# soedinglab/PEnG-motif

Measured on AMD Instinct MI355X. Metric: 4^W pattern z-scores/s + EM PWM-kmer evals/s at W=10; Gbp/s k-mer count, higher is better.
Workload: dtype u32 counts / f32 scores / f32 serial EM sums (f64 tree sums in the throughput EM mode)

## Files before the change

peng-motif_amd/csrc/em.hip:

```cpp
#include "em_serial.h"

namespace pengk {
namespace {
#ifdef PENGK_WG_TRACE
constexpr unsigned WG_TRACE_MAX = 1u << 20;
__device__ unsigned long long g_wg_trace[3 * WG_TRACE_MAX];
__device__ unsigned g_wg_trace_n;
struct WgTrace {
  unsigned long long t0;
  unsigned kernel;
  __device__ __forceinline__ WgTrace(unsigned k) : t0(__builtin_amdgcn_s_memrealtime()), kernel(k) {}
  __device__ __forceinline__ void end(unsigned kind, unsigned wg) const {
    if (threadIdx.x != 0) return;
    const unsigned long long t1 = __builtin_amdgcn_s_memrealtime();
    const unsigned xcc = __builtin_amdgcn_s_getreg((4 << 11) | (0 << 6) | 20) & 0xFu;
    const unsigned i = atomicAdd(&g_wg_trace_n, 1u);
    if (i < WG_TRACE_MAX) {
      g_wg_trace[3 * i] = ((unsigned long long)kernel << 56) | ((unsigned long long)kind << 48) | ((unsigned long long)xcc << 40) | wg;
      g_wg_trace[3 * i + 1] = t0;
      g_wg_trace[3 * i + 2] = t1;
    }
  }
};
#define PENGK_WG_TRACE_BEGIN(k) const WgTrace wg_trace(k)
// ... 347 lines not shown
    constexpr bool LEAN = decltype(lean_tag)::value;
#pragma unroll 1
    for (uint32_t d6 = 0; d6 < 4u; ++d6) {
#pragma unroll
      for (uint32_t d5 = 0; d5 < 4u; ++d5) {
        float s5 = 0.0f;
#pragma unroll
        for (uint32_t d4 = 0; d4 < 4u; ++d4) {
          const uint32_t xl = t + 256u * (d4 + 4u * d5 + 16u * d6);
          float pr = ((p3 * f4_[d4]) * f5_[d5]) * f6_[d6];
#pragma unroll
          for (int p = 7; p < W; ++p) pr = pr * hi[p - 7];
          const float odds = em_div<LEAN>(pr, bgs[xl]);
          const float v = em_div<LEAN>((float)cnt[xl] * saturation, 1 + em_div<LEAN>(saturation, odds));
          out[xl] = v;
          flagged |= __float_as_uint(v) > 0x7F7FFFFFu;
          c4[d4] += v;
          s5 += v;
        }
        c5[d5] += s5;
        c6[d6] += s5;
      }
    }
  };
  if (lean) body(std::true_type{});
  else body(std::false_type{});
  if (flagged) bad[pw] = 1u;
  const float tot = (c6[0] + c6[1]) + (c6[2] + c6[3]);
  auto all = [](float v) {
#pragma unroll
    for (int m = 1; m < 64; m <<= 1) v += __shfl_xor(v, m, 64);
    return v;
  };
#pragma unroll
  for (int a = 0; a < 4; ++a) {
    const float s4 = all(c4[a]), s5 = all(c5[a]), s6 = all(c6[a]);
    if (lane == 0) {
      part[wave][12 + a] = s4;
      part[wave][16 + a] = s5;
      part[wave][20 + a] = s6;
    }
  }
#pragma unroll
  for (int d = 0; d < 3; ++d) {
    float v = tot;
#pragma unroll
    for (int m = 1; m < 64; m <<= 1)
      if (m != (1 << (2 * d)) && m != (2 << (2 * d))) v += __shfl_xor(v, m, 64);
    if ((lane & ~(3u << (2 * d))) == 0u) part[wave][4 * d + (lane >> (2 * d))] = v;
  }
  {
    const float v = all(tot);
    if (lane == 0) part[wave][24] = v;
  }
  __syncthreads();
  if (t < G::CELLS) {
    const uint32_t p = t >> 2, a = t & 3u;
    float* o = sums + (size_t)pw * G::CELLS * G::NBLK;
    if (p <= 6u) {
      float v;
      if (p == 3u) v = part[a][24];
      else {
        const uint32_t at = p <= 2u ? 4u * p + a : 4u * (p - 1u) + a;
        v = (part[0][at] + part[1][at]) + (part[2][at] + part[3][at]);
      }
      o[(size_t)t * G::NBLK + sp] = v;
    } else {
      const float v = (part[0][20 + a] + part[1][20 + a]) + (part[2][20 + a] + part[3][20 + a]);
      o[(size_t)(4u * p + G::high_digit(p, sp)) * G::NBLK + G::high_block(p, sp, a)] = v;
    }
  }
  PENGK_WG_TRACE_END(0, blockIdx.x + gridDim.x * blockIdx.y);
}

template <int W>
__global__ __launch_bounds__(64) void em_block_predict_kernel(const uint32_t* __restrict__ run_now, const uint32_t* __restrict__ bad,
                                                              const float* __restrict__ sums, seqsum::BlockRecord* __restrict__ rec,
                                                              uint32_t skew) {
  using G = BlockGeo<W>;
  const uint32_t pw = blockIdx.y, cell = blockIdx.x, lane = threadIdx.x;
  if (run_now[pw] == 0u || bad[pw]) return;
  constexpr uint32_t PER = G::NBLK / 64u;
  static_assert(G::NBLK % 64u == 0u, "whole lanes");
  const float* in = sums + ((size_t)pw * G::CELLS + cell) * G::NBLK + (size_t)lane * PER;
  seqsum::BlockRecord* out = rec + ((size_t)pw * G::CELLS + cell) * G::NBLK + (size_t)lane * PER;
  double mine = 0.0;
  for (uint32_t i = 0; i < PER; ++i) mine += (double)in[i];
  double before = mine;
#pragma unroll
  for (int d = 1; d < 64; d <<= 1) {
    const double o = __shfl_up(before, d, 64);
    if ((int)lane >= d) before += o;
  }
  before -= mine;
  for (uint32_t i = 0; i < PER; ++i) {
    const double after = before + (double)in[i];
    const uint32_t e = block_binade(before, after, skew, cell * G::NBLK + lane * PER + i);
    seqsum::BlockRecord r;
    r.e = e;
    r.d0 = 0.0f;
    r.d1 = 0.0f;
    r.pad = 0u;
    out[i] = r;
    before = after;
  }
}

constexpr uint32_t SPAN_EVAL_WAVES = 8;
template <int W>
__global__ __launch_bounds__(64 * SPAN_EVAL_WAVES) void em_span_eval_kernel(const uint32_t* __restrict__ run_now, const float* __restrict__ wbuf,
                                                                            seqsum::BlockRecord* __restrict__ rec,
                                                                            const uint32_t* __restrict__ bad, uint32_t n_pwm,
                                                                            const float* __restrict__ sums, uint32_t skew,
                                                                            uint32_t extra_wgs, uint32_t head_blocks) {
  using G = BlockGeo<W>;
  PENGK_WG_TRACE_BEGIN(2);
  const uint32_t lin = blockIdx.x + gridDim.x * blockIdx.y;
  __shared__ __attribute__((aligned(16))) float span[16384];
  const uint32_t t = threadIdx.x, lane = t & 63u;
  const uint32_t wave = (uint32_t)__builtin_amdgcn_readfirstlane((int)(t >> 6));
  if (lin < extra_wgs) {
    constexpr uint32_t XW = (G::CELLS + 3u) / 4u;
    uint32_t pw, xunit;
    if (!group_map(lin, n_pwm, XW, pw, xunit)) return;
    const uint32_t cell = 4u * xunit + wave;
    if (wave >= 4u || cell >= G::CELLS || run_now[pw] == 0u || bad[pw]) return;
    seqsum::lds_float* buf = (seqsum::lds_float*)span + wave * seqsum::BLOCK;
    const float* w = wbuf + (size_t)pw * G::NP;
    seqsum::Row mine;
    seqsum::Stats st;
    float s0 = 0.0f;
    const bool first_position = (cell >> 2) == 0u;
    auto stage = [&](uint32_t b) {
      uint32_t l = lane;
      asm volatile("" : "+v"(l));
      if (first_position) {
        EmTerms0<W> src0{w, cell & 3u};
        src0.bind_stage(l);
        src0.stage(b, l, buf);
      } else {
        EmTerms<W> src{w, cell >> 2, cell & 3u};
        src.bind_stage(l);
        src.stage(b, l, buf);
      }
    };
    stage(0u);
#pragma unroll 1
    for (uint32_t b = 0; b < head_blocks; ++b) {
      asm volatile("s_waitcnt vmcnt(0)" ::: "memory");
      mine.read_staged(buf, lane);
      asm volatile("s_waitcnt lgkmcnt(0)" ::: "memory");
      if (b + 1u < head_blocks) stage(b + 1u);
      s0 = seqsum::fold_block(mine, lane, s0, st);
    }
    if (lane == 0) {
      seqsum::BlockRecord out;
      out.e = seqsum::SUM_BEHIND;
      out.d0 = s0;
      out.d1 = 0.0f;
      out.pad = head_blocks;
      rec[((size_t)pw * G::CELLS + cell) * G::NBLK] = out;
    }
    PENGK_WG_TRACE_END(1, lin);
    return;
  }
  uint32_t pw, sp;
  if (!group_map(lin - extra_wgs, n_pwm, G::SPANS, pw, sp)) return;
  constexpr uint32_t T = 64u * SPAN_EVAL_WAVES, PER = 4096u / T;
  seqsum::f4 v[PER];
  {
    const seqsum::f4* src = reinterpret_cast<const seqsum::f4*>(wbuf + (size_t)pw * G::NP + (size_t)sp * 16384u);
#pragma unroll
    for (uint32_t k = 0; k < PER; ++k) v[k] = src[t + T * k];
  }
  const uint32_t running = run_now[pw];
  const uint32_t flagged = bad[pw];
  constexpr uint32_t TASKS = (G::CELLS + SPAN_EVAL_WAVES - 1u) / SPAN_EVAL_WAVES;
  seqsum::BlockRecord* cells = rec + (size_t)pw * G::CELLS * G::NBLK;
  auto cell_of = [&](uint32_t task) { return (task >> 2) <= 6u ? task : 4u * (task >> 2) + G::high_digit(task >> 2, sp); };
  auto block_of = [&](uint32_t task) { return (task >> 2) <= 6u ? sp : G::high_block(task >> 2, sp, task & 3u); };
  uint32_t binades = seqsum::NO_BINADE;
  if constexpr (G::PREDICT_IN_EVAL) {
    constexpr uint32_t LOADS = G::NBLK / 64u, GROUP = LOADS <= 4u ? TASKS : 2u;
#pragma unroll 1
    for (uint32_t i0 = 0; i0 < TASKS; i0 += GROUP) {
      float part[GROUP], own[GROUP];
#pragma unroll
      for (uint32_t g = 0; g < GROUP; ++g) {
        const uint32_t task = min(wave + SPAN_EVAL_WAVES * (i0 + g), G::CELLS - 1u);
        const uint32_t cell = cell_of(task), b = block_of(task);
        const float* cs = sums + ((size_t)pw * G::CELLS + cell) * G::NBLK;
        float acc = 0.0f;
#pragma unroll
        for (uint32_t c = 0; c < G::NBLK; c += 64u) {
          const float x = cs[c + lane];
          acc += c + lane < b ? x : 0.0f;
        }
        part[g] = acc;
        own[g] = cs[b];
      }
#pragma unroll
      for (uint32_t g = 0; g < GROUP; ++g) {
        const uint32_t i = i0 + g, task = wave + SPAN_EVAL_WAVES * i;
        float acc = part[g];
#pragma unroll
        for (int m = 1; m < 64; m <<= 1) acc += __shfl_xor(acc, m, 64);
        if (i < TASKS && task < G::CELLS) {
          const uint32_t e = block_binade((double)acc, (double)acc + (double)own[g], skew, cell_of(task) * G::NBLK + block_of(task));
          if (lane == i) binades = e;
        }
      }
    }
  } else {
#pragma unroll 1
    for (uint32_t i = 0; i < TASKS; ++i) {
      const uint32_t task = wave + SPAN_EVAL_WAVES * i;
      if (task < G::CELLS) {
        const uint32_t e = cells[(size_t)cell_of(task) * G::NBLK + block_of(task)].e;
        if (lane == i) binades = e;
      }
    }
  }
  if (running == 0 || flagged) return;
  {
    seqsum::f4* dst = reinterpret_cast<seqsum::f4*>(span);
#pragma unroll
    for (uint32_t k = 0; k < PER; ++k) {
      const uint32_t idx = t + T * k;
      dst[SpanLds::slot_of(idx >> 4, idx & 15u)] = v[k];
    }
  }
  __syncthreads();
  PENGK_WG_TRACE_END(2, lin);
#pragma unroll 1
  for (uint32_t task = wave, i = 0; task < G::CELLS; task += SPAN_EVAL_WAVES, ++i) {
    const uint32_t p = task >> 2, j = task & 3u;
    if (block_of(task) < head_blocks) continue;
    seqsum::BlockRecord* r = cells + (size_t)cell_of(task) * G::NBLK + block_of(task);
    const uint32_t e = (uint32_t)__builtin_amdgcn_readlane((int)binades, (int)i);
    if (e == seqsum::NO_BINADE) {
      if (G::PREDICT_IN_EVAL && lane == 0) r->e = seqsum::NO_BINADE;
      continue;
    }
    seqsum::Row mine;
    span_row<W>(span, p, j, lane, mine);
    float d0, d1;
    const bool ok = seqsum::block_increments(mine, lane, seqsum::bases_of_binade(e), d0, d1);
    if (lane == 0) {
      seqsum::BlockRecord out;
      out.e = ok ? e : seqsum::NO_BINADE;
      out.d0 = d0;
      out.d1 = d1;
      out.pad = 0u;
      *r = out;
    }
  }
  PENGK_WG_TRACE_END(0, lin);
}

template <int W>
__global__ __launch_bounds__(64) void em_chain_store_kernel(const uint32_t* __restrict__ run, const uint32_t* __restrict__ bad,
                                                            const float* __restrict__ wbuf, const seqsum::BlockRecord* __restrict__ rec,
                                                            float* __restrict__ cellsum, uint32_t n_pwm,
                                                            unsigned long long* __restrict__ counters) {
  using G = BlockGeo<W>;
  PENGK_WG_TRACE_BEGIN(3);
  const uint32_t lin = blockIdx.x + gridDim.x * blockIdx.y;
  uint32_t pw, cell;
  if (!group_map(lin, n_pwm, G::CELLS, pw, cell)) return;
  __shared__ __attribute__((aligned(16))) float lds[seqsum::WALK_LDS_FLOATS];
  seqsum::WalkCounts wc;
  const uint32_t lane = threadIdx.x;
  const seqsum::BlockRecord* r = rec + ((size_t)pw * G::CELLS + cell) * G::NBLK;
  uint32_t running = run[pw];
  uint32_t flagged = bad[pw];
  uint4 first = reinterpret_cast<const uint4*>(r)[lane];
  asm volatile("" : "+s"(running), "+s"(flagged), "+v"(first.x), "+v"(first.y), "+v"(first.z), "+v"(first.w));
  if (running == 0u) return;
  float s = 0.0f;
  const float* w = wbuf + (size_t)pw * G::NP;
  if (flagged) {
    const uint32_t p = cell >> 2, a = cell & 3u;
    for (uint32_t c = 0; c < (1u << (2 * W - 2)); ++c)
      s += w[((c >> (2u * p)) << (2u * p + 2u)) | (a << (2u * p)) | (c & ((1u << (2u * p)) - 1u))];
  } else if ((cell >> 2) == 0u) {
    EmTerms0<W> src0{w, cell & 3u};
    src0.bind_stage(lane);
    s = seqsum::walk_chain(src0, r, first, G::NBLK, (seqsum::lds_float*)lds, lane, wc);
  } else {
    EmTerms<W> src{w, cell >> 2, cell & 3u};
    src.bind_stage(lane);
    s = seqsum::walk_chain(src, r, first, G::NBLK, (seqsum::lds_float*)lds, lane, wc);
  }
  if (lane == 0) {
    cellsum[(size_t)pw * G::CELLS + cell] = s;
    if (wc.fetched) __hip_atomic_fetch_add(counters + 0, (unsigned long long)wc.fetched, __ATOMIC_RELAXED, __HIP_MEMORY_SCOPE_AGENT);
    if (wc.mispredicted) __hip_atomic_fetch_add(counters + 1, (unsigned long long)wc.mispredicted, __ATOMIC_RELAXED, __HIP_MEMORY_SCOPE_AGENT);
    if (wc.restaged) __hip_atomic_fetch_add(counters + 2, (unsigned long long)wc.restaged, __ATOMIC_RELAXED, __HIP_MEMORY_SCOPE_AGENT);
    if (wc.restaged_waits) __hip_atomic_fetch_add(counters + 3, (unsigned long long)wc.restaged_waits, __ATOMIC_RELAXED, __HIP_MEMORY_SCOPE_AGENT);
  }
  PENGK_WG_TRACE_END(wc.fetched > 255u ? 255u : wc.fetched, lin);
}

template <int W>
__global__ __launch_bounds__(64) void em_serial_finish_kernel(FusedState fs, uint32_t K, float threshold, int max_it) {
  constexpr uint32_t CELLS = 4u * W;
  const uint32_t pw = blockIdx.x, t = threadIdx.x;
  __shared__ __attribute__((aligned(16))) float s_pwm[CELLS], s_old[CELLS];
  const uint32_t running = fs.run[(size_t)((K - 1u) & 1u) * fs.run_stride + pw];
  if (running) {
    const float* prev = ((K - 1u) & 1u) ? fs.pwm1 : fs.pwm0;
    if (t < CELLS) {
      s_old[t] = prev[(size_t)pw * CELLS + t];
      s_pwm[t] = fs.cellsum[(size_t)pw * CELLS + t];
    }
    __syncthreads();
    const float change = finalize_rows<W>(s_pwm, s_old, t);
    if (t < CELLS) fs.pwm0[(size_t)pw * CELLS + t] = s_pwm[t];
    if (t == 0) {
      fs.state[2 * pw] = (int)K;
      fs.state[2 * pw + 1] = !(change <= threshold || (int)K >= max_it);
      fs.change[pw] = change;
    }
  } else {
    const int it = fs.state[2 * pw];
    if ((it & 1) && t < CELLS) fs.pwm0[(size_t)pw * CELLS + t] = fs.pwm1[(size_t)pw * CELLS + t];
  }
  if (t == 0) {
    fs.bad[pw] = 0u;
    fs.bad[(size_t)fs.bad_stride + pw] = 0u;
  }
}

__global__ __launch_bounds__(256) void em_serial_setup_kernel(uint32_t n, int W, float threshold, int max_it, int32_t* __restrict__ state,
                                                             float* __restrict__ change, uint32_t* __restrict__ run,
                                                             unsigned long long* __restrict__ counters, uint32_t* __restrict__ bg_range,
                                                             uint32_t lean, uint32_t* __restrict__ bad, uint32_t bad_words) {
  const uint32_t i = blockIdx.x * 256u + threadIdx.x;
  if (i < (uint32_t)EM_COUNTERS) counters[i] = 0ull;
  if (i == 0) {
    bg_range[0] = lean ? 0xFFFFFFFFu : 0u;
    bg_range[1] = lean ? 0u : 0xFFFFFFFFu;
  }
  for (uint32_t j = i; j < bad_words; j += gridDim.x * 256u) bad[j] = 0u;
  if (i >= n) return;
  const float c0 = (float)W;
  const uint32_t r = !(c0 <= threshold || 0 >= max_it);
  state[2 * i] = 0;
  state[2 * i + 1] = (int32_t)r;
  change[i] = c0;
  run[i] = r;
  run[n + i] = r;
}

template <int W, int HIMAX, bool FAST, int P>
int launch_geo(pengk_ctx* ctx, int64_t n_pwm, float* d_pwms, float saturation, float threshold, int max_it,
               const uint32_t* d_counts, const float* d_bg, int32_t* d_state, float* d_change) {
  using G = EmGeo<W, HIMAX>;
  hipLaunchKernelGGL(em_init_kernel, dim3((unsigned)((n_pwm + 255) / 256)), dim3(256), 0, ctx->stream, (int)n_pwm, W, threshold,
                     max_it, d_state, d_change);
  PENGK_HIP(hipGetLastError());
  const size_t per_pwm = (size_t)G::NB * G::CELLS * sizeof(double);
  const size_t budget = (size_t)256 << 20;
  int64_t batch = (int64_t)(budget / per_pwm);
  if (batch < 1) batch = 1;
  if (batch > n_pwm) batch = n_pwm;
  if (batch > 65535) batch = 65535;
  if (batch > P) batch -= batch % P;
  int rc = ensure_scratch(ctx, (void**)&ctx->d_em_partials, &ctx->em_partials_bytes, (size_t)batch * per_pwm);
  if (rc) return rc;
  if (FAST) {
    const uint32_t np = 1u << (2 * W);
    rc = ensure_scratch(ctx, (void**)&ctx->d_em_tables, &ctx->em_tables_bytes, (size_t)2 * np * sizeof(float));
    if (rc) return rc;
    float* cs = ctx->d_em_tables;
    float* sb = cs + np;
    const unsigned pb = (np + 255) / 256 < 4096u ? (np + 255) / 256 : 4096u;
    hipLaunchKernelGGL(em_prepare_kernel, dim3(pb), dim3(256), 0, ctx->stream, d_counts, d_bg, saturation, np, cs, sb);
    PENGK_HIP(hipGetLastError());
    d_counts = reinterpret_cast<const uint32_t*>(cs);
    d_bg = sb;
  }
  for (int64_t first = 0; first < n_pwm; first += batch) {
    const int64_t nb = n_pwm - first < batch ? n_pwm - first : batch;
    for (int it = 0; it < max_it; ++it) {
      hipLaunchKernelGGL((em_accumulate_kernel<W, HIMAX, FAST, P>), dim3(G::NB, (unsigned)((nb + P - 1) / P)), dim3(256), 0,
                         ctx->stream, d_pwms + (size_t)first * W * 4, d_state + 2 * first, d_counts, d_bg, saturation,
                         ctx->d_em_partials, (int)nb);
      hipLaunchKernelGGL((em_finalize_kernel<W, HIMAX>), dim3((unsigned)nb), dim3(64), 0, ctx->stream,
                         d_pwms + (size_t)first * W * 4, d_state + 2 * first, d_change + first, ctx->d_em_partials, threshold, max_it,
                         (uint32_t*)nullptr, (const float*)nullptr, 0u);
    }
    PENGK_HIP(hipGetLastError());
  }
  return PENGK_OK;
}

#ifdef PENGK_WG_TRACE
}
}
extern "C" __attribute__((visibility("default"))) long long pengk_debug_wg_trace(unsigned long long* out, unsigned max) {
  unsigned n = 0;
  if (hipDeviceSynchronize() != hipSuccess) return -1;
  if (hipMemcpyFromSymbol(&n, HIP_SYMBOL(pengk::g_wg_trace_n), sizeof n) != hipSuccess) return -1;
  const unsigned m = n < max ? n : max;
  if (m && hipMemcpyFromSymbol(out, HIP_SYMBOL(pengk::g_wg_trace), (size_t)m * 3 * sizeof(unsigned long long)) != hipSuccess) return -1;
  const unsigned zero = 0;
  if (hipMemcpyToSymbol(HIP_SYMBOL(pengk::g_wg_trace_n), &zero, sizeof zero) != hipSuccess) return -1;
  return (long long)n;
}
namespace pengk {
namespace {
#endif

#ifdef PENGK_SEQSUM_STATS
}
}
extern "C" __attribute__((visibility("default"))) int pengk_debug_seqsum_stats(unsigned long long* out, int reset) {
  if (hipMemcpyFromSymbol(out, HIP_SYMBOL(pengk::seqsum::g_stats), 12 * sizeof(unsigned long long)) != hipSuccess) return 1;
  if (reset) {
    unsigned long long z[12] = {0};
    if (hipMemcpyToSymbol(HIP_SYMBOL(pengk::seqsum::g_stats), z, sizeof z) != hipSuccess) return 1;
  }
  return 0;
}
namespace pengk {
namespace {
#endif

template <int W>
int launch_serial_ahead(pengk_ctx* ctx, int64_t n_pwm, float* d_pwms, float saturation, float threshold, int max_it,
                        const uint32_t* d_counts, const float* d_bg, int32_t* d_state, float* d_change, size_t budget, bool split) {
  using B = BlockGeo<W>;
  using LG = LookGeo<W>;
  const size_t np = (size_t)1 << (2 * W);
  int lanes = ctx->em_overlap < 1 ? 1 : ctx->em_overlap > MAX_EM_LANES ? MAX_EM_LANES : ctx->em_overlap;
  while (lanes > 1 && n_pwm < 8 * (int64_t)lanes) --lanes;
  const int64_t fit = std::max<int64_t>(1, (int64_t)(budget / lanes / (np * sizeof(float))));
  int64_t batch = fit;
  if (batch * lanes > n_pwm) {
    batch = lanes > 1 ? ((n_pwm + lanes - 1) / lanes + 7) / 8 * 8 : n_pwm;
    if (batch > fit) batch = fit >= 8 ? fit / 8 * 8 : fit;
  }
  if (batch > 16384) batch = 16384;
  const size_t tables_b = (size_t)batch * np * sizeof(float);
  const size_t sums_b = split ? ((size_t)batch * B::CELLS * B::NBLK * sizeof(float) + 255) / 256 * 256 : 0;
  const size_t rec_b = sums_b + ((size_t)batch * B::CELLS * B::NBLK * sizeof(seqsum::BlockRecord) + 255) / 256 * 256;
  const size_t look_b = split ? 0 : ((size_t)batch * LG::WORDS_PER_PWM * sizeof(unsigned long long) + 255) / 256 * 256;
  const size_t flags_at = ((size_t)batch * B::CELLS * sizeof(float) + 255) / 256 * 256;
  const size_t small_b = (flags_at + (size_t)2 * batch * sizeof(uint32_t) + 255) / 256 * 256;
  const size_t run_at = lanes * small_b;
  const size_t pwm1_at = (run_at + (size_t)2 * n_pwm * sizeof(uint32_t) + 255) / 256 * 256;
  int rc = ensure_scratch(ctx, (void**)&ctx->d_em_tables, &ctx->em_tables_bytes, lanes * tables_b);
  if (rc) return rc;
  rc = ensure_scratch(ctx, (void**)&ctx->d_em_partials, &ctx->em_partials_bytes, pwm1_at + (size_t)n_pwm * B::CELLS * sizeof(float));
  if (rc) return rc;
  rc = ensure_scratch(ctx, &ctx->d_em_blocks, &ctx->em_blocks_bytes, lanes * rec_b);
  if (rc) return rc;
  if (look_b) {
    const size_t had = ctx->em_look_bytes;
    rc = ensure_scratch(ctx, &ctx->d_em_look, &ctx->em_look_bytes, lanes * look_b);
    if (rc) return rc;
    if (ctx->em_look_bytes != had || ctx->em_epoch >= 0xFFFF0000u) {
      PENGK_HIP(hipStreamSynchronize(ctx->stream));
      for (int l = 0; l < MAX_EM_LANES - 1; ++l)
        if (ctx->em_streams[l]) PENGK_HIP(hipStreamSynchronize(ctx->em_streams[l]));
      PENGK_HIP(hipMemsetAsync(ctx->d_em_look, 0, ctx->em_look_bytes, ctx->stream));
      ctx->em_epoch = 0;
    }
  }
  if (!ctx->d_em_counters) PENGK_HIP(hipMalloc((void**)&ctx->d_em_counters, (EM_COUNTERS + 1) * sizeof(unsigned long long)));
  uint32_t* bg_range = reinterpret_cast<uint32_t*>(ctx->d_em_counters + EM_COUNTERS);
  char* small = reinterpret_cast<char*>(ctx->d_em_partials);
  uint32_t* run = reinterpret_cast<uint32_t*>(small + run_at);
  float* pwm1 = reinterpret_cast<float*>(small + pwm1_at);
  {
    const uint32_t words = (uint32_t)((run_at - flags_at) / sizeof(uint32_t));
    hipLaunchKernelGGL(em_serial_setup_kernel, dim3((unsigned)((std::max<int64_t>(n_pwm, 1024) + 255) / 256)), dim3(256), 0, ctx->stream,
                       (uint32_t)n_pwm, W, threshold, max_it, d_state, d_change, run, ctx->d_em_counters, bg_range,
                       ctx->em_lean_div ? 1u : 0u, reinterpret_cast<uint32_t*>(small + flags_at), words);
    if (ctx->em_lean_div)
      hipLaunchKernelGGL(em_bg_range_kernel, dim3(32), dim3(1024), 0, ctx->stream, d_bg, (uint32_t)np, bg_range);
    PENGK_HIP(hipGetLastError());
  }
  if (max_it <= 0) return PENGK_OK;
  hipStream_t streams[MAX_EM_LANES];
  streams[0] = ctx->stream;
  for (int l = 1; l < lanes; ++l) {
    if (!ctx->em_streams[l - 1]) PENGK_HIP(hipStreamCreateWithFlags(&ctx->em_streams[l - 1], hipStreamNonBlocking));
    if (!ctx->em_join[l - 1]) PENGK_HIP(hipEventCreateWithFlags(&ctx->em_join[l - 1], hipEventDisableTiming));
    streams[l] = ctx->em_streams[l - 1];
  }
  if (lanes > 1 && !ctx->em_fork) PENGK_HIP(hipEventCreateWithFlags(&ctx->em_fork, hipEventDisableTiming));
  if (lanes > 1) {
    PENGK_HIP(hipEventRecord(ctx->em_fork, ctx->stream));
    for (int l = 1; l < lanes; ++l) PENGK_HIP(hipStreamWaitEvent(streams[l], ctx->em_fork, 0));
  }
  const int rc_launch = [&]() -> int {
    for (int64_t round0 = 0; round0 < n_pwm; round0 += batch * lanes) {
      for (int it = 1; it <= max_it + 1; ++it) {
        for (int l = 0; l < lanes; ++l) {
          const int64_t first = round0 + (int64_t)l * batch;
          if (first >= n_pwm) break;
          const int64_t nb = n_pwm - first < batch ? n_pwm - first : batch;
          hipStream_t st = streams[l];
          float* tables = reinterpret_cast<float*>(reinterpret_cast<char*>(ctx->d_em_tables) + l * tables_b);
          float* sums = reinterpret_cast<float*>(reinterpret_cast<char*>(ctx->d_em_blocks) + l * rec_b);
          seqsum::BlockRecord* rec = reinterpret_cast<seqsum::BlockRecord*>(reinterpret_cast<char*>(ctx->d_em_blocks) + l * rec_b + sums_b);
          unsigned long long* look = reinterpret_cast<unsigned long long*>(reinterpret_cast<char*>(ctx->d_em_look) + l * look_b);
          float* cellsum = reinterpret_cast<float*>(small + l * small_b);
          uint32_t* bad = reinterpret_cast<uint32_t*>(small + l * small_b + flags_at);
          FusedState fs;
          fs.run = run + first;
          fs.pwm0 = d_pwms + (size_t)first * W * 4;
          fs.pwm1 = pwm1 + (size_t)first * W * 4;
          fs.bad = bad;
          fs.cellsum = cellsum;
          fs.state = d_state + 2 * first;
          fs.change = d_change + first;
          fs.n = (uint32_t)nb;
          fs.run_stride = (uint32_t)n_pwm;
          fs.bad_stride = (uint32_t)batch;
          if (it > max_it) {
            hipLaunchKernelGGL((em_serial_finish_kernel<W>), dim3((unsigned)nb), dim3(64), 0, st, fs, (uint32_t)max_it, threshold, max_it);
            continue;
          }
          const uint32_t k = (uint32_t)it;
          const unsigned groups = (unsigned)((nb + 7) / 8 * 8);
          const uint32_t* run_now = run + (size_t)((k - 1u) & 1u) * n_pwm + first;
          const uint32_t* bad_now = bad + (size_t)(k & 1u) * batch;
          if (split) {
            hipLaunchKernelGGL((em_weights_span_kernel<W>), dim3(B::SPANS, (unsigned)nb), dim3(256), 0, st, d_counts, d_bg, saturation, tables,
                               sums, (const uint32_t*)bg_range, fs, k, threshold, max_it);
            if (!B::PREDICT_IN_EVAL)
              hipLaunchKernelGGL((em_block_predict_kernel<W>), dim3(B::CELLS, (unsigned)nb), dim3(64), 0, st, run_now, bad_now,
                                 (const float*)sums, rec, (uint32_t)ctx->em_test_skew);
            const uint64_t xwgs = (uint64_t)nb * ((B::CELLS + 3) / 4), swgs = xwgs + (uint64_t)nb * B::SPANS;
            hipLaunchKernelGGL((em_span_eval_kernel<W>), dim3(1024u, (unsigned)((swgs + 1023u) / 1024u)), dim3(64 * SPAN_EVAL_WAVES), 0, st,
                               run_now, (const float*)tables, rec, bad_now, (uint32_t)nb, (const float*)sums,
                               (uint32_t)ctx->em_test_skew, (uint32_t)xwgs, (uint32_t)std::min<uint64_t>(ctx->em_head_blocks, B::NBLK));
            hipLaunchKernelGGL((em_chain_store_kernel<W>), dim3((unsigned)(4 * W), (unsigned)nb), dim3(64), 0, st, run_now, bad_now,
                               (const float*)tables, (const seqsum::BlockRecord*)rec, cellsum, (uint32_t)nb, ctx->d_em_counters);
            continue;
          }
          if constexpr (LG::SUPPORTED) {
            const uint64_t wgs = (uint64_t)groups * B::SPANS;
            const unsigned gx = 1024u;
            const uint32_t epoch = ++ctx->em_epoch;
            const int rc_fused = launch_span_fused(W, gx, (unsigned)((wgs + gx - 1) / gx), st, fs, k, threshold, max_it, d_counts, d_bg, saturation,
                                                   tables, rec, look, epoch, (const uint32_t*)bg_range, (uint32_t)ctx->em_test_skew,
                                                   (uint32_t)ctx->em_test_lookback);
            if (rc_fused) return rc_fused;
          }
          hipLaunchKernelGGL((em_chain_store_kernel<W>), dim3((unsigned)(4 * W), (unsigned)nb), dim3(64), 0, st, run_now, bad_now,
                             (const float*)tables, (const seqsum::BlockRecord*)rec, cellsum, (uint32_t)nb, ctx->d_em_counters);
        }
      }
      PENGK_HIP(hipGetLastError());
    }
    return PENGK_OK;
  }();
  int rc_join = PENGK_OK;
  for (int l = 1; l < lanes; ++l) {
    hipError_t e = hipEventRecord(ctx->em_join[l - 1], streams[l]);
    if (e == hipSuccess) e = hipStreamWaitEvent(ctx->stream, ctx->em_join[l - 1], 0);
    if (e != hipSuccess) {
      (void)hipStreamSynchronize(streams[l]);
      if (!rc_join) rc_join = hip_fail(e, "joining the EM's streams");
    }
  }
  return rc_launch ? rc_launch : rc_join;
}

#ifndef PENGK_EM_BUDGET_GIB
// ... 150 lines not shown
```

peng-motif_amd/csrc/seqsum.h:

```cpp
#pragma once
#include <hip/hip_runtime.h>
#include <stdint.h>

namespace pengk {
namespace seqsum {

constexpr uint32_t SEG = 64;
constexpr uint32_t BLOCK = 64 * SEG;
constexpr uint32_t SEG_STRIDE = SEG + 4;
constexpr uint32_t LDS_FLOATS = 64 * SEG_STRIDE;
constexpr uint32_t INF_BITS = 0x7F800000u;

typedef float f4 __attribute__((ext_vector_type(4)));
typedef __attribute__((address_space(3))) float lds_float;
typedef __attribute__((address_space(3))) f4 lds_f4;

#ifdef PENGK_SEQSUM_STATS
__device__ unsigned long long g_stats[12];
struct Stats {
  unsigned long long v[12] = {0, 0, 0, 0, 0, 0, 0, 0, 0, 0, 0, 0};
  __device__ __forceinline__ void flush(uint32_t lane) {
    if (lane == 0)
      for (int i = 0; i < 12; ++i) atomicAdd(&g_stats[i], v[i]);
  }
};
#define PENGK_STAT_ADD(i, x) do { st.v[i] += (unsigned long long)(x); } while (0)
#define PENGK_CLOCK() __builtin_amdgcn_s_memtime()
#else
struct Stats {
  __device__ __forceinline__ void flush(uint32_t) {}
};
#define PENGK_STAT_ADD(i, x) do { } while (0)
#define PENGK_CLOCK() 0ull
#endif

__device__ __forceinline__ uint32_t bits(float v) { return __float_as_uint(v); }

struct Bases {
  float b0, b1;
  uint32_t limit;
};
__device__ __forceinline__ Bases bases_of(float s) {
  const uint32_t e = bits(s) >> 23;
  Bases r;
  if (e <= 1u) {
    r.b0 = 0.0f;
    r.b1 = __uint_as_float(1u);
    r.limit = 2u << 23;
  } else {
    r.b0 = __uint_as_float(e << 23);
    r.b1 = __uint_as_float((e << 23) | 1u);
    r.limit = (e + 1u) << 23;
  }
  return r;
}

__device__ __forceinline__ void compose(float& a0, float& a1, float b0, float b1, const Bases& B) {
  const float d0 = b0 - B.b0, d1 = b1 - B.b1;
  a0 = a0 + ((bits(a0) & 1u) ? d1 : d0);
  a1 = a1 + ((bits(a1) & 1u) ? d1 : d0);
}

struct Row {
  f4 q[SEG / 4u];
  __device__ __forceinline__ void read(const float* row) {
    const f4* src = reinterpret_cast<const f4*>(row);
#pragma unroll
    for (uint32_t j = 0; j < SEG / 4u; ++j) q[j] = src[j];
    static_assert(SEG == 64u, "sixteen quads");
    asm volatile("" : "+v"(q[0]), "+v"(q[1]), "+v"(q[2]), "+v"(q[3]), "+v"(q[4]), "+v"(q[5]), "+v"(q[6]), "+v"(q[7]), "+v"(q[8]),
                 "+v"(q[9]), "+v"(q[10]), "+v"(q[11]), "+v"(q[12]), "+v"(q[13]), "+v"(q[14]), "+v"(q[15]));
  }
  __device__ __forceinline__ void read_staged(const lds_float* buf, uint32_t l) {
    const lds_f4* src = (const lds_f4*)buf + 16u * l;
#pragma unroll
    for (uint32_t j = 0; j < SEG / 4u; ++j) q[j] = src[j ^ (l & 15u)];
    asm volatile("" : "+v"(q[0]), "+v"(q[1]), "+v"(q[2]), "+v"(q[3]), "+v"(q[4]), "+v"(q[5]), "+v"(q[6]), "+v"(q[7]), "+v"(q[8]),
                 "+v"(q[9]), "+v"(q[10]), "+v"(q[11]), "+v"(q[12]), "+v"(q[13]), "+v"(q[14]), "+v"(q[15]));
  }
#define PENGK_ADD2(T) "v_add_f32 %0, " T ", %0\n\tv_add_f32 %1, " T ", %1\n\t"
#define PENGK_ADD1(T) "v_add_f32 %0, " T ", %0\n\t"
  static __device__ __forceinline__ void add16x2(float& x0, float& x1, const f4& a, const f4& b, const f4& c, const f4& d) {
    asm(PENGK_ADD2("%2") PENGK_ADD2("%3") PENGK_ADD2("%4") PENGK_ADD2("%5") PENGK_ADD2("%6") PENGK_ADD2("%7") PENGK_ADD2("%8")
        PENGK_ADD2("%9") PENGK_ADD2("%10") PENGK_ADD2("%11") PENGK_ADD2("%12") PENGK_ADD2("%13") PENGK_ADD2("%14")
        PENGK_ADD2("%15") PENGK_ADD2("%16") PENGK_ADD2("%17")
        : "+v"(x0), "+v"(x1)
        : "v"(a.x), "v"(a.y), "v"(a.z), "v"(a.w), "v"(b.x), "v"(b.y), "v"(b.z), "v"(b.w), "v"(c.x), "v"(c.y), "v"(c.z), "v"(c.w),
          "v"(d.x), "v"(d.y), "v"(d.z), "v"(d.w));
  }
  static __device__ __forceinline__ void add16(float& x, const f4& a, const f4& b, const f4& c, const f4& d) {
    asm(PENGK_ADD1("%1") PENGK_ADD1("%2") PENGK_ADD1("%3") PENGK_ADD1("%4") PENGK_ADD1("%5") PENGK_ADD1("%6") PENGK_ADD1("%7")
        PENGK_ADD1("%8") PENGK_ADD1("%9") PENGK_ADD1("%10") PENGK_ADD1("%11") PENGK_ADD1("%12") PENGK_ADD1("%13")
        PENGK_ADD1("%14") PENGK_ADD1("%15") PENGK_ADD1("%16")
        : "+v"(x)
        : "v"(a.x), "v"(a.y), "v"(a.z), "v"(a.w), "v"(b.x), "v"(b.y), "v"(b.z), "v"(b.w), "v"(c.x), "v"(c.y), "v"(c.z), "v"(c.w),
          "v"(d.x), "v"(d.y), "v"(d.z), "v"(d.w));
  }
#undef PENGK_ADD2
#undef PENGK_ADD1
  __device__ __forceinline__ void run2(float& x0, float& x1) const {
#pragma unroll
    for (uint32_t j = 0; j < SEG / 4u; j += 4u) add16x2(x0, x1, q[j], q[j + 1u], q[j + 2u], q[j + 3u]);
  }
  __device__ __forceinline__ float run1(float x) const {
#pragma unroll
    for (uint32_t j = 0; j < SEG / 4u; j += 4u) add16(x, q[j], q[j + 1u], q[j + 2u], q[j + 3u]);
    return x;
  }
};

template <int D>
__device__ __forceinline__ float row_shr(float self, float v) {
  return __int_as_float(__builtin_amdgcn_update_dpp(__float_as_int(self), __float_as_int(v), 0x110 + D, 0xf, 0xf, false));
}
__device__ __forceinline__ float lane_value(float v, int l) {
  return __int_as_float(__builtin_amdgcn_readlane(__float_as_int(v), l));
}

__device__ __forceinline__ float ends_behind(float i0, float i1, const Bases& B, float s, uint32_t lane) {
  const uint32_t par = bits(s) & 1u;
  const uint32_t rw = lane >> 4;
  float end;
  const float d0 = i0 - B.b0, d1 = i1 - B.b1;
  if (__builtin_amdgcn_ballot_w64(bits(d0) != bits(d1)) == 0ull) {
    float d = d0;
    d += row_shr<1>(0.0f, d);
    d += row_shr<2>(0.0f, d);
    d += row_shr<4>(0.0f, d);
    d += row_shr<8>(0.0f, d);
    d += __int_as_float(__builtin_amdgcn_update_dpp(0, __float_as_int(d), 0x142 , 0xa, 0xf, false));
    d += __int_as_float(__builtin_amdgcn_update_dpp(0, __float_as_int(d), 0x143 , 0xc, 0xf, false));
    end = s + d;
  } else {
#define PENGK_ROW_STEP(D)                                                     \
    {                                                                        \
      float a0 = row_shr<D>(B.b0, i0), a1 = row_shr<D>(B.b1, i1);            \
      compose(a0, a1, i0, i1, B);                                            \
      i0 = a0;                                                               \
      i1 = a1;                                                               \
    }
    PENGK_ROW_STEP(1) PENGK_ROW_STEP(2) PENGK_ROW_STEP(4) PENGK_ROW_STEP(8)
#undef PENGK_ROW_STEP
    float p0 = lane_value(i0, 15), p1 = lane_value(i1, 15);
    float q0 = p0, q1 = p1;
    compose(q0, q1, lane_value(i0, 31), lane_value(i1, 31), B);
    float r0 = q0, r1 = q1;
    compose(r0, r1, lane_value(i0, 47), lane_value(i1, 47), B);
    float f0 = rw == 1u ? p0 : rw == 2u ? q0 : rw == 3u ? r0 : B.b0;
    float f1 = rw == 1u ? p1 : rw == 2u ? q1 : rw == 3u ? r1 : B.b1;
    compose(f0, f1, i0, i1, B);
    end = s + (par ? f1 - B.b1 : f0 - B.b0);
  }
  return end;
}

__device__ __forceinline__ float fold_block(const Row& mine, uint32_t lane, float s, Stats& st) {
  uint32_t first = 0;
  for (;;) {
    PENGK_STAT_ADD(1, 1);
    const unsigned long long k2 = PENGK_CLOCK();
    if (bits(s) >= INF_BITS) return s;
    const Bases B = bases_of(s);
    float i0 = B.b0, i1 = B.b1;
    mine.run2(i0, i1);
#ifdef PENGK_SEQSUM_STATS
    asm volatile("" : "+v"(i0), "+v"(i1));
#endif
    const unsigned long long k3 = PENGK_CLOCK();
    PENGK_STAT_ADD(5, k3 - k2);
    if (lane < first) {
      i0 = B.b0;
      i1 = B.b1;
    }
    const float end = ends_behind(i0, i1, B, s, lane);
    const unsigned long long flagged = __builtin_amdgcn_ballot_w64(bits(end) >= B.limit);
    const unsigned long long k4 = PENGK_CLOCK();
    PENGK_STAT_ADD(6, k4 - k3);
    if (!flagged) return lane_value(end, 63);
    const int L = __builtin_ctzll(flagged);
    float v = s;
    if (L > 0) v = lane_value(end, L - 1);
    s = lane_value(mine.run1(v), L);
    first = (uint32_t)L + 1u;
#ifdef PENGK_SEQSUM_STATS
    asm volatile("" : "+v"(s));
#endif
    PENGK_STAT_ADD(7, PENGK_CLOCK() - k4);
    if (first == 64u) return s;
  }
}

constexpr uint32_t NO_BINADE = 0xFFFFFFFFu;
constexpr uint32_t SUM_BEHIND = 0xFFFFFFFEu;
__device__ __forceinline__ uint32_t binade_of(float s) {
  const uint32_t e = bits(s) >> 23;
  return e <= 1u ? 1u : e;
}
__device__ __forceinline__ Bases bases_of_binade(uint32_t e) {
  Bases r;
  r.b0 = __uint_as_float(e <= 1u ? 0u : e << 23);
  r.b1 = __uint_as_float(e <= 1u ? 1u : (e << 23) | 1u);
  r.limit = (e + 1u) << 23;
  return r;
}

__device__ __forceinline__ bool block_increments(const Row& mine, uint32_t lane, const Bases& B, float& D0, float& D1) {
  float i0 = B.b0, i1 = B.b1;
  mine.run2(i0, i1);
  const uint32_t rw = lane >> 4;
  const float d0 = i0 - B.b0, d1 = i1 - B.b1;
  float x0, x1;
  if (__builtin_amdgcn_ballot_w64(bits(d0) != bits(d1)) == 0ull) {
    float d = d0;
    d += row_shr<1>(0.0f, d);
    d += row_shr<2>(0.0f, d);
    d += row_shr<4>(0.0f, d);
    d += row_shr<8>(0.0f, d);
    d += __int_as_float(__builtin_amdgcn_update_dpp(0, __float_as_int(d), 0x142 , 0xa, 0xf, false));
    d += __int_as_float(__builtin_amdgcn_update_dpp(0, __float_as_int(d), 0x143 , 0xc, 0xf, false));
    x0 = B.b0 + d;
    x1 = B.b1 + d;
  } else {
#define PENGK_ROW_STEP(D)                                                     \
    {                                                                          \
      float a0 = row_shr<D>(B.b0, i0), a1 = row_shr<D>(B.b1, i1);              \
      compose(a0, a1, i0, i1, B);                                              \
      i0 = a0;                                                                 \
      i1 = a1;                                                                 \
    }
    PENGK_ROW_STEP(1) PENGK_ROW_STEP(2) PENGK_ROW_STEP(4) PENGK_ROW_STEP(8)
#undef PENGK_ROW_STEP
    float p0 = lane_value(i0, 15), p1 = lane_value(i1, 15);
    float q0 = p0, q1 = p1;
    compose(q0, q1, lane_value(i0, 31), lane_value(i1, 31), B);
    float r0 = q0, r1 = q1;
    compose(r0, r1, lane_value(i0, 47), lane_value(i1, 47), B);
    float f0 = rw == 1u ? p0 : rw == 2u ? q0 : rw == 3u ? r0 : B.b0;
    float f1 = rw == 1u ? p1 : rw == 2u ? q1 : rw == 3u ? r1 : B.b1;
    compose(f0, f1, i0, i1, B);
    x0 = f0;
    x1 = f1;
  }
  x0 = lane_value(x0, 63);
  x1 = lane_value(x1, 63);
  D0 = x0 - B.b0;
  D1 = x1 - B.b1;
  return bits(x0) < B.limit && bits(x1) < B.limit;
}

struct BlockRecord {
  uint32_t e;
  float d0, d1;
  uint32_t pad;
};

constexpr uint32_t WALK_LDS_FLOATS = 2u * BLOCK;
#ifdef PENGK_TEST_WALK_RACE
#define PENGK_WALK_RESTAGED(x) false
#else
#define PENGK_WALK_RESTAGED(x) (x)
#endif
template <uint32_t N>
__device__ __forceinline__ void wait_loads_but() {
  static_assert(N == 0u || N == 16u, "the counts walk_chain needs");
  if (N == 0u)
    asm volatile("s_waitcnt vmcnt(0)" ::: "memory");
  else
    asm volatile("s_waitcnt vmcnt(16)" ::: "memory");
}
struct WalkCounts {
  uint32_t fetched = 0, mispredicted = 0, restaged = 0, restaged_waits = 0;
};
template <class Source>
__device__ __forceinline__ float walk_chain(const Source& src, const BlockRecord* __restrict__ rec, const uint4& first_records,
                                            uint32_t n_blocks, lds_float* lds, uint32_t lane, WalkCounts& wc) {
  Stats st;
  const unsigned long long w0 = PENGK_CLOCK();
  float s = 0.0f;
  lds_float* bufa = lds;
  lds_float* bufb = lds + BLOCK;
  uint32_t ha = NO_BINADE, hb = NO_BINADE;
  bool a_first = true;
  bool restaged = false;
  uint4 r_next = first_records;
#pragma unroll 1
  for (uint32_t base = 0; base < n_blocks; base += 64u) {
    const uint4 r = r_next;
    if (base + 64u < n_blocks) r_next = reinterpret_cast<const uint4*>(rec)[base + 64u + lane];
    unsigned long long open = __builtin_amdgcn_ballot_w64(r.x == NO_BINADE);
    auto open_after = [&](uint32_t b) {
      const uint32_t j = b - base;
      const unsigned long long rest = j < 63u ? open & ~((2ull << j) - 1ull) : 0ull;
      return rest ? base + (uint32_t)__builtin_ctzll(rest) : NO_BINADE;
    };
    uint32_t j = 0;
    if (base == 0u && (uint32_t)__builtin_amdgcn_readfirstlane((int)r.x) == SUM_BEHIND) {
      s = __uint_as_float((uint32_t)__builtin_amdgcn_readfirstlane((int)r.y));
      j = (uint32_t)__builtin_amdgcn_readfirstlane((int)r.w);
      j = j < 1u ? 1u : j > 64u ? 64u : j;
      open = j < 64u ? open & ~((1ull << j) - 1ull) : 0ull;
    }
    if (open) {
      ha = base + (uint32_t)__builtin_ctzll(open);
      src.stage(ha, lane, bufa);
      hb = open_after(ha);
      if (hb != NO_BINADE) src.stage(hb, lane, bufb);
      a_first = true;
      restaged = false;
    }
#pragma unroll 1
    while (j < 64u) {
      const uint32_t e = binade_of(s);
      const unsigned long long same = __builtin_amdgcn_ballot_w64(r.x == e) >> j;
      const uint32_t len = same == ~0ull ? 64u : (uint32_t)__builtin_ctzll(~same);
      if (len != 0u && bits(s) < INF_BITS) {
        const Bases B = bases_of_binade(e);
        const bool in = lane >= j && lane < j + len;
        const float end = ends_behind(in ? B.b0 + __uint_as_float(r.y) : B.b0, in ? B.b1 + __uint_as_float(r.z) : B.b1, B, s, lane);
        const unsigned long long flagged = __builtin_amdgcn_ballot_w64(in && bits(end) >= B.limit);
        if (!flagged) {
          s = lane_value(end, (int)(j + len - 1u));
          j += len;
          continue;
        }
        const uint32_t L = (uint32_t)__builtin_ctzll(flagged);
        if (L > j) s = lane_value(end, (int)(L - 1u));
        j = L;
      }
      const uint32_t b = base + j;
      const unsigned long long c0 = PENGK_CLOCK();
      Row mine;
#define PENGK_TAKE(buf1, h1, h2)                                                          \
      {                                                                                   \
        const bool ahead = h1 == b;                                                       \
        if (!ahead) {                                                                     \
          src.stage(b, lane, buf1);                                                       \
          wait_loads_but<0u>();                                                           \
          PENGK_STAT_ADD(9, 1);                                                           \
          ++wc.mispredicted;                                                              \
        } else if (h2 != NO_BINADE && !PENGK_WALK_RESTAGED(restaged) && Source::STAGE_LOADS == 16u) { \
          wait_loads_but<16u>();                                                          \
        } else {                                                                          \
          wc.restaged_waits += (h2 != NO_BINADE && restaged) ? 1u : 0u;                   \
          wait_loads_but<0u>();                                                           \
        }                                                                                 \
        mine.read_staged(buf1, lane);                                                     \
        asm volatile("s_waitcnt lgkmcnt(0)" ::: "memory");                                \
        if (ahead) {                                                                      \
          h1 = open_after(h2 != NO_BINADE ? h2 : b);                                      \
          a_first = !a_first;                                                             \
          restaged = false;                                                               \
        } else {                                                                          \
          restaged = h1 != NO_BINADE;  \
          wc.restaged += restaged ? 1u : 0u;                                              \
        }                                                                                 \
        if (h1 != NO_BINADE) src.stage(h1, lane, buf1);                                   \
      }
      if (a_first) PENGK_TAKE(bufa, ha, hb) else PENGK_TAKE(bufb, hb, ha)
#undef PENGK_TAKE
      const unsigned long long c1 = PENGK_CLOCK();
      PENGK_STAT_ADD(2, c1 - c0);
      s = fold_block(mine, lane, s, st);
#ifdef PENGK_SEQSUM_STATS
      asm volatile("" : "+v"(s));
#endif
      PENGK_STAT_ADD(3, PENGK_CLOCK() - c1);
      PENGK_STAT_ADD(0, 1);
      ++wc.fetched;
      ++j;
    }
  }
#ifdef PENGK_SEQSUM_STATS
  asm volatile("" : "+v"(s));
#endif
  PENGK_STAT_ADD(8, PENGK_CLOCK() - w0);
  PENGK_STAT_ADD(10, 1);
  st.flush(lane);
  asm volatile("s_waitcnt vmcnt(0)" ::: "memory");
  return s;
}

__device__ __forceinline__ void lds_barrier() { asm volatile("s_waitcnt lgkmcnt(0)\n\ts_barrier" ::: "memory"); }

#ifndef PENGK_FETCH_WAVES
#define PENGK_FETCH_WAVES 1
#endif
constexpr uint32_t FETCH_WAVES = PENGK_FETCH_WAVES;
constexpr uint32_t CHAIN_THREADS = 64u * (1u + FETCH_WAVES);
constexpr uint32_t CHAIN_LDS_FLOATS = LDS_FLOATS + 4u;
template <class Source, bool CHECK>
__device__ __forceinline__ float fold_chain(const Source& src, uint32_t n_blocks, float* lds, uint32_t thread) {
  const uint32_t lane = thread & 63u;
  const uint32_t wave = (uint32_t)__builtin_amdgcn_readfirstlane((int)(thread >> 6));
  const bool fetcher = wave != 0u;
  const uint32_t q = wave - 1u;
  volatile uint32_t* bad = reinterpret_cast<volatile uint32_t*>(lds + LDS_FLOATS);
  if (CHECK) {
    if (thread == 0) *bad = 0u;
    __syncthreads();
  }
  Stats st;
  float s = 0.0f;
  bool fallback = false;
  if (fetcher) {
    float R[64];
    if (q < n_blocks) src.template load<1>(q, 0u, lane, R);
#pragma unroll 1
    for (uint32_t i = 0; i < n_blocks; ++i) {
      if (i % FETCH_WAVES == q) {
        if (CHECK) {
          uint32_t m = 0;
#pragma unroll
          for (int k = 0; k < 64; ++k) m = max(m, bits(R[k]));
          if (__builtin_amdgcn_ballot_w64(m > 0x7F7FFFFFu) && lane == 0) *bad = 1u;
        }
        const unsigned long long c0 = PENGK_CLOCK();
        src.template deposit<1>(0u, lane, R, lds);
        if (i + FETCH_WAVES < n_blocks) src.template load<1>(i + FETCH_WAVES, 0u, lane, R);
        PENGK_STAT_ADD(2, PENGK_CLOCK() - c0);
      }
      lds_barrier();
      if (CHECK && *bad) break;
      lds_barrier();
    }
  } else {
#pragma unroll 1
    for (uint32_t i = 0; i < n_blocks; ++i) {
      lds_barrier();
      if (CHECK && *bad) {
        fallback = true;
        break;
      }
      const unsigned long long k0 = PENGK_CLOCK();
      Row mine;
      mine.read(lds + lane * SEG_STRIDE);
      PENGK_STAT_ADD(4, PENGK_CLOCK() - k0);
      lds_barrier();
      const unsigned long long c0 = PENGK_CLOCK();
      s = fold_block(mine, lane, s, st);
      PENGK_STAT_ADD(0, 1);
      PENGK_STAT_ADD(3, PENGK_CLOCK() - c0);
    }
    if (CHECK && fallback) s = src.serial();
  }
  st.flush(lane);
  return fetcher ? 0.0f : s;
}

}
}
```

Before: 587.8.

## Add binade-run fast path to serial block fold after first mismatch

After the first flagged lane, fold_block now predicts each later lane's binade from the neighbouring partial sums. It precomputes a single run2 pass at that binade and then resolves whole stretches of consecutive same-binade lanes with one ends_behind scan, instead of restarting the full block pass or stepping lane by lane. The aim is to cut the repeated full-block recomputation and serial run1 steps when a block crosses binades. The tail loop path is explicitly kept on the old behaviour through fold_block<false>. The head path uses the new ROWS variant, which adds more ballot and DPP logic and a possible extra run2 pass. Stats plumbing grows to 16 counters.

Result: no change. 591.0 (median of 6 runs) (+0.6%).

```diff
diff --git a/peng-motif_amd/csrc/em.hip b/peng-motif_amd/csrc/em.hip
--- a/peng-motif_amd/csrc/em.hip
+++ b/peng-motif_amd/csrc/em.hip
@@ -523,7 +523,13 @@
       asm volatile("s_waitcnt lgkmcnt(0)" ::: "memory");
       if (b + 1u < head_blocks) stage(b + 1u);
       s0 = seqsum::fold_block(mine, lane, s0, st);
-    }
+#ifdef PENGK_SEQSUM_STATS_HEADS
+      PENGK_STAT_ADD(0, 1);
+#endif
+    }
+#ifdef PENGK_SEQSUM_STATS_HEADS
+    st.flush(lane);
+#endif
     if (lane == 0) {
       seqsum::BlockRecord out;
       out.e = seqsum::SUM_BEHIND;
@@ -788,9 +794,9 @@
 }
 }
 extern "C" __attribute__((visibility("default"))) int pengk_debug_seqsum_stats(unsigned long long* out, int reset) {
-  if (hipMemcpyFromSymbol(out, HIP_SYMBOL(pengk::seqsum::g_stats), 12 * sizeof(unsigned long long)) != hipSuccess) return 1;
+  if (hipMemcpyFromSymbol(out, HIP_SYMBOL(pengk::seqsum::g_stats), pengk::seqsum::N_STATS * sizeof(unsigned long long)) != hipSuccess) return 1;
   if (reset) {
-    unsigned long long z[12] = {0};
+    unsigned long long z[pengk::seqsum::N_STATS] = {0};
     if (hipMemcpyToSymbol(HIP_SYMBOL(pengk::seqsum::g_stats), z, sizeof z) != hipSuccess) return 1;
   }
   return 0;
diff --git a/peng-motif_amd/csrc/seqsum.h b/peng-motif_amd/csrc/seqsum.h
--- a/peng-motif_amd/csrc/seqsum.h
+++ b/peng-motif_amd/csrc/seqsum.h
@@ -16,12 +16,13 @@
 typedef __attribute__((address_space(3))) f4 lds_f4;
 
 #ifdef PENGK_SEQSUM_STATS
-__device__ unsigned long long g_stats[12];
+constexpr int N_STATS = 16;
+__device__ unsigned long long g_stats[N_STATS];
 struct Stats {
-  unsigned long long v[12] = {0, 0, 0, 0, 0, 0, 0, 0, 0, 0, 0, 0};
+  unsigned long long v[N_STATS] = {0, 0, 0, 0, 0, 0, 0, 0, 0, 0, 0, 0, 0, 0, 0, 0};
   __device__ __forceinline__ void flush(uint32_t lane) {
     if (lane == 0)
-      for (int i = 0; i < 12; ++i) atomicAdd(&g_stats[i], v[i]);
+      for (int i = 0; i < N_STATS; ++i) atomicAdd(&g_stats[i], v[i]);
   }
 };
 #define PENGK_STAT_ADD(i, x) do { st.v[i] += (unsigned long long)(x); } while (0)
@@ -154,21 +155,46 @@
   return end;
 }
 
+constexpr uint32_t NO_BINADE = 0xFFFFFFFFu;
+__device__ __forceinline__ uint32_t binade_of(float s) {
+  const uint32_t e = bits(s) >> 23;
+  return e <= 1u ? 1u : e;
+}
+__device__ __forceinline__ Bases bases_of_binade(uint32_t e) {
+  Bases r;
+  r.b0 = __uint_as_float(e <= 1u ? 0u : e << 23);
+  r.b1 = __uint_as_float(e <= 1u ? 1u : (e << 23) | 1u);
+  r.limit = (e + 1u) << 23;
+  return r;
+}
+__device__ __forceinline__ float lane_before(float self, float v) {
+  return __int_as_float(__builtin_amdgcn_update_dpp(__float_as_int(self), __float_as_int(v), 0x138 , 0xf, 0xf, false));
+}
+__device__ __forceinline__ uint32_t row_binade(float before, float after) {
+  const float lo = before * (1.0f - 1.0f / 65536.0f), hi = after * (1.0f + 1.0f / 65536.0f);
+  const uint32_t e = binade_of(lo);
+  return bits(hi) < 0x7F000000u && e == binade_of(hi) ? e : NO_BINADE;
+}
+
+template <bool ROWS = true>
 __device__ __forceinline__ float fold_block(const Row& mine, uint32_t lane, float s, Stats& st) {
-  uint32_t first = 0;
+  float i0, i1;
+  uint32_t mine_e = NO_BINADE;
+  uint32_t r = 0;
   for (;;) {
     PENGK_STAT_ADD(1, 1);
     const unsigned long long k2 = PENGK_CLOCK();
     if (bits(s) >= INF_BITS) return s;
     const Bases B = bases_of(s);
-    float i0 = B.b0, i1 = B.b1;
+    i0 = B.b0;
+    i1 = B.b1;
     mine.run2(i0, i1);
 #ifdef PENGK_SEQSUM_STATS
     asm volatile("" : "+v"(i0), "+v"(i1));
 #endif
     const unsigned long long k3 = PENGK_CLOCK();
     PENGK_STAT_ADD(5, k3 - k2);
-    if (lane < first) {
+    if (lane < r) {
       i0 = B.b0;
       i1 = B.b1;
     }
@@ -178,31 +204,67 @@
     PENGK_STAT_ADD(6, k4 - k3);
     if (!flagged) return lane_value(end, 63);
     const int L = __builtin_ctzll(flagged);
-    float v = s;
-    if (L > 0) v = lane_value(end, L - 1);
-    s = lane_value(mine.run1(v), L);
-    first = (uint32_t)L + 1u;
+    if (ROWS) mine_e = (int)lane > L ? row_binade(lane_before(s, end), end) : NO_BINADE;
+    if (L > 0) s = lane_value(end, L - 1);
+    s = lane_value(mine.run1(s), L);
+    r = (uint32_t)L + 1u;
 #ifdef PENGK_SEQSUM_STATS
     asm volatile("" : "+v"(s));
 #endif
     PENGK_STAT_ADD(7, PENGK_CLOCK() - k4);
-    if (first == 64u) return s;
-  }
-}
-
-constexpr uint32_t NO_BINADE = 0xFFFFFFFFu;
+    PENGK_STAT_ADD(11, 1);
+    if (r == 64u) return s;
+    if (ROWS) break;
+  }
+  if (bits(s) >= INF_BITS) return s;
+  {
+    PENGK_STAT_ADD(1, 1);
+    PENGK_STAT_ADD(13, 1);
+    const unsigned long long k3 = PENGK_CLOCK();
+    const Bases P = bases_of_binade(mine_e == NO_BINADE ? 1u : mine_e);
+    i0 = P.b0;
+    i1 = P.b1;
+    mine.run2(i0, i1);
+#ifdef PENGK_SEQSUM_STATS
+    asm volatile("" : "+v"(i0), "+v"(i1));
+#endif
+    PENGK_STAT_ADD(5, PENGK_CLOCK() - k3);
+  }
+  for (;;) {
+    const uint32_t e = binade_of(s);
+    const unsigned long long same = __builtin_amdgcn_ballot_w64(mine_e == e) >> r;
+    const uint32_t len = (uint32_t)__builtin_ctzll(~same);
+    if (len != 0u) {
+      PENGK_STAT_ADD(12, 1);
+      const unsigned long long k5 = PENGK_CLOCK();
+      const Bases B = bases_of_binade(e);
+      const bool in = lane >= r && lane < r + len;
+      const float end = ends_behind(in ? i0 : B.b0, in ? i1 : B.b1, B, s, lane);
+      const unsigned long long flagged = __builtin_amdgcn_ballot_w64(in && bits(end) >= B.limit);
+      PENGK_STAT_ADD(6, PENGK_CLOCK() - k5);
+      if (!flagged) {
+        s = lane_value(end, (int)(r + len - 1u));
+        r += len;
+        if (r == 64u) return s;
+      } else {
+        const uint32_t L = (uint32_t)__builtin_ctzll(flagged);
+        if (L > r) s = lane_value(end, (int)L - 1);
+        r = L;
+      }
+    }
+    const unsigned long long k4 = PENGK_CLOCK();
+    s = lane_value(mine.run1(s), (int)r);
+    ++r;
+#ifdef PENGK_SEQSUM_STATS
+    asm volatile("" : "+v"(s));
+#endif
+    PENGK_STAT_ADD(7, PENGK_CLOCK() - k4);
+    PENGK_STAT_ADD(11, 1);
+    if (r == 64u || bits(s) >= INF_BITS) return s;
+  }
+}
+
 constexpr uint32_t SUM_BEHIND = 0xFFFFFFFEu;
-__device__ __forceinline__ uint32_t binade_of(float s) {
-  const uint32_t e = bits(s) >> 23;
-  return e <= 1u ? 1u : e;
-}
-__device__ __forceinline__ Bases bases_of_binade(uint32_t e) {
-  Bases r;
-  r.b0 = __uint_as_float(e <= 1u ? 0u : e << 23);
-  r.b1 = __uint_as_float(e <= 1u ? 1u : (e << 23) | 1u);
-  r.limit = (e + 1u) << 23;
-  return r;
-}
 
 __device__ __forceinline__ bool block_increments(const Row& mine, uint32_t lane, const Bases& B, float& D0, float& D1) {
   float i0 = B.b0, i1 = B.b1;
@@ -360,7 +422,7 @@
 #undef PENGK_TAKE
       const unsigned long long c1 = PENGK_CLOCK();
       PENGK_STAT_ADD(2, c1 - c0);
-      s = fold_block(mine, lane, s, st);
+      s = fold_block<false>(mine, lane, s, st);
 #ifdef PENGK_SEQSUM_STATS
       asm volatile("" : "+v"(s));
 #endif
@@ -375,7 +437,9 @@
 #endif
   PENGK_STAT_ADD(8, PENGK_CLOCK() - w0);
   PENGK_STAT_ADD(10, 1);
+#ifndef PENGK_SEQSUM_STATS_HEADS
   st.flush(lane);
+#endif
   asm volatile("s_waitcnt vmcnt(0)" ::: "memory");
   return s;
 }
```
